# PytorchConnectomics/pytorch_connectomics

Hardware: AMD Instinct MI355X
Metric: voxels/s (train + sliding-window infer), MedNeXt-S 112^3 bf16 (higher is better)
Workload: dtype bf16; 1 GPU; Lucchi++ sliding-window inference (configs[1]): MedNeXt-S k3, 165x1024x768 volume, roi 112^3, overlap 0.5, bump blending, sw_batch_size 8, random-init weights; step = one whole-volume EagerSlidingWindowEngine call (TTA off); value = window-voxels/s; sw_batch_size=8, window_pipeline_streams=3

## Files before the change

### pytorch_connectomics_amd/csrc/pw_common.h

```cpp
#pragma once
#include "pytc_common.h"

namespace pytc {

template <typename TW>
struct Mma;

template <>
struct Mma<bf16_t> {
  static constexpr int EPL = 8;
  static constexpr int KSTEP = 32;
  typedef bf16x8_t frag_t;
  static __device__ __forceinline__ f32x4_t mma(frag_t a, frag_t b, f32x4_t c) {
    return __builtin_amdgcn_mfma_f32_16x16x32_bf16(a, b, c, 0, 0, 0);
  }
  static __device__ __forceinline__ frag_t from_floats(const float (&v)[8]) {
    f32x8_t f;
#pragma unroll
    for (int i = 0; i < 8; ++i) f[i] = v[i];
    return __builtin_convertvector(f, frag_t);
  }
};

template <>
// ... 79 lines not shown
    } else if (full) VecIO<TO, NCH>::load(resn + off, rv);
    else {
#pragma unroll
      for (int i = 0; i < NCH; ++i) rv[i] = (o0 + i < C_out) ? to_f32<TO>(resn[off + i]) : 0.f;
    }
    const float* cf = e.res_bias + (long)n * 3 * C_out + o0;
#pragma unroll
    for (int i = 0; i < NCH; ++i)
      if (o0 + i < C_out) v[i] = fmaf(cf[i], v[i], fmaf(cf[C_out + i], rv[i], cf[2 * C_out + i]));
    if (e.Go_w > 0) {
      const unsigned ur = (unsigned)orow, gw = (unsigned)e.Go_w, gh = (unsigned)e.Go_h;
      const unsigned tq = ur / gw;
      const int px = (int)(ur - tq * gw), pz = (int)(tq / gh), py = (int)(tq - (unsigned)pz * gh);
      if (px == 0 || py == 0 || pz == 0) return;
      const long crow = ((long)(pz - 1) * (e.Go_h - 1) + (py - 1)) * (e.Go_w - 1) + (px - 1);
      TO* yc = reinterpret_cast<TO*>(e.y) + ((long)n * (e.Go_d - 1) * (e.Go_h - 1) * (e.Go_w - 1) + crow) * C_out + o0;
      if (full) VecIO<TO, NCH>::store(yc, v);
      else {
#pragma unroll
        for (int i = 0; i < NCH; ++i)
          if (o0 + i < C_out) yc[i] = from_f32<TO>(v[i]);
      }
      return;
    }
  } else if (e.res_mode == PYTC_RES_UPSAMPLE) {
    int px, py, pz;
    if (pos) { pz = pos[0]; py = pos[1]; px = pos[2]; }
    else {
      const unsigned ur = (unsigned)orow, gw = (unsigned)e.Go_w, gh = (unsigned)e.Go_h;
      const unsigned t = ur / gw;
      px = (int)(ur - t * gw);
      pz = (int)(t / gh);
      py = (int)(t - (unsigned)pz * gh);
    }
    float sk[NCH];
    if (pre) {
#pragma unroll
      for (int i = 0; i < NCH; ++i) sk[i] = pre[i];
    } else if (full) VecIO<TO, NCH>::load(resn + off, sk);
    else {
#pragma unroll
      for (int i = 0; i < NCH; ++i) sk[i] = (o0 + i < C_out) ? to_f32<TO>(resn[off + i]) : 0.f;
    }
    if (px == 0 || py == 0 || pz == 0) {
#pragma unroll
      for (int i = 0; i < NCH; ++i) v[i] = sk[i];
    } else {
      const int oz = pz - 1, oy = py - 1, ox = px - 1;
      float rl[NCH];
      if (e.res_low && !((oz | oy | ox) & 1)) {
        const TO* rp = reinterpret_cast<const TO*>(e.res_low) +
                       ((((long)n * e.Gl_d + (oz >> 1)) * e.Gl_h + (oy >> 1)) * e.Gl_w + (ox >> 1)) * C_out + o0;
        if (full) VecIO<TO, NCH>::load(rp, rl);
        else {
#pragma unroll
          for (int i = 0; i < NCH; ++i) rl[i] = (o0 + i < C_out) ? to_f32<TO>(rp[i]) : 0.f;
        }
      } else {
#pragma unroll
        for (int i = 0; i < NCH; ++i) rl[i] = (e.res_bias && o0 + i < C_out) ? e.res_bias[o0 + i] : 0.f;
      }
#pragma unroll
      for (int i = 0; i < NCH; ++i) v[i] = v[i] + rl[i] + sk[i];
    }
  }
  if (full) {
    if constexpr (sizeof(TO) == 2 && NCH == 8) {
      if (e.nt) {
        f32x8_t f;
#pragma unroll
        for (int i = 0; i < 8; ++i) f[i] = v[i];
        __builtin_nontemporal_store(__builtin_convertvector(f, bf16x8_t), reinterpret_cast<bf16x8_t*>(yn + off));
        return;
      }
    }
    VecIO<TO, NCH>::store(yn + off, v);
  } else {
#pragma unroll
    for (int i = 0; i < NCH; ++i)
      if (o0 + i < C_out) yn[off + i] = from_f32<TO>(v[i]);
  }
}

template <typename TI, int EPL>
__device__ __forceinline__ void load_row_frag(const TI* __restrict__ row, int k0, int C_in, bool vec_ok,
                                              float (&v)[EPL]) {
  if (vec_ok && k0 + EPL <= C_in) {
    if constexpr (sizeof(TI) == 4 && EPL == 8) {
      float t0[4], t1[4];
      VecIO<float, 4>::load(reinterpret_cast<const float*>(row) + k0, t0);
      VecIO<float, 4>::load(reinterpret_cast<const float*>(row) + k0 + 4, t1);
#pragma unroll
      for (int i = 0; i < 4; ++i) { v[i] = t0[i]; v[4 + i] = t1[i]; }
    } else {
      VecIO<TI, EPL>::load(row + k0, v);
    }
  } else {
#pragma unroll
    for (int j = 0; j < EPL; ++j) v[j] = (k0 + j < C_in) ? to_f32<TI>(row[k0 + j]) : 0.f;
  }
}

template <int PER>
struct WarmRegs { unsigned int r[2 * PER]; };
template <int PER>
__device__ __forceinline__ void warm_l2(const void* base, long bytes, WarmRegs<PER>& w, int first) {
  const long lines = (bytes + 127) >> 7;
  const long lin = (long)blockIdx.z * gridDim.y * gridDim.x + (long)blockIdx.y * gridDim.x + blockIdx.x;
  const long total = (long)gridDim.x * gridDim.y * gridDim.z;
  const long per_xcd = (total + 7) >> 3;
  const long stride = per_xcd * blockDim.x;
  long l = (lin >> 3) * blockDim.x + threadIdx.x;
#pragma unroll
  for (int it = 0; it < PER; ++it, l += stride) {
    const long lc = l < lines ? l : lines - 1;
    const char* ptr = reinterpret_cast<const char*>(base) + (lc << 7);
    asm volatile("global_load_dword %0, %1, off" : "=v"(w.r[first + it]) : "v"(ptr) : "memory");
  }
}
template <int PER>
__device__ __forceinline__ void warm_l2_done(WarmRegs<PER>& w) {
  asm volatile("s_waitcnt vmcnt(0)" : : : "memory");
#pragma unroll
  for (int i = 0; i < 2 * PER; ++i) asm volatile("" : : "v"(w.r[i]) : "memory");
}

__device__ __forceinline__ float apply_act(float t, int act) {
  if (act == PYTC_ACT_GELU) return gelu_erf(t);
  if (act == PYTC_ACT_SIGMOID) return 1.f / (1.f + __expf(-t));
  if (act == PYTC_ACT_TANH) return tanhf(t);
  return t;
}

}
```

### pytorch_connectomics_amd/csrc/pw_mlp_chunk_kernels.hip

```cpp
#include "pw_common.h"

namespace pytc {

struct MlpChunkParams {
  const bf16_t* t;
  const float* ab;
  const bf16x8_t* w2;
  const float* b2;
  const h8_t* w3;
  const float* b3;
  EpiParams e;
  long rps;
  int N, C_in, C_hid, C_out, HC;
  long w2_stride;
};

__device__ __forceinline__ void chunk_glds16(const void* gsrc, unsigned lds_dst) {
  unsigned keep;
  asm volatile("s_mov_b32 %0, m0\n\ts_mov_b32 m0, %2\n\ts_nop 0\n\tglobal_load_lds_dwordx4 %1, off\n\ts_mov_b32 m0, %0"
               : "=&s"(keep) : "v"(gsrc), "s"(lds_dst) : "memory");
}

template <int KS_IN, int MO, int NW, int WPS>
__global__ void __launch_bounds__(NW * 64, WPS)
pw_mlp_chunk_kernel(MlpChunkParams p) {
  constexpr int NT = 2, CIN = KS_IN * 32, COUT = MO * 16;
  constexpr int PIECES = 2 * KS_IN + MO;
  constexpr int MINE = (PIECES + NW - 1) / NW;
  constexpr int NBUF = 3;
  extern __shared__ __attribute__((aligned(16))) unsigned char chunk_lds[];
  uint4* ring = reinterpret_cast<uint4*>(chunk_lds);
  float* lb2 = reinterpret_cast<float*>(chunk_lds + (size_t)NBUF * PIECES * 1024);
  float* lb3 = lb2 + p.C_hid;
  const int tid = threadIdx.x, lane = tid & 63;
  const int wave = __builtin_amdgcn_readfirstlane(tid >> 6);
  const int r = lane & 15, kb = lane >> 4;
  const int n = blockIdx.y;
  const bool folded = p.ab == nullptr;
  const long row0 = ((long)blockIdx.x * NW + wave) * (NT * 16);
  const bool with_res = p.e.res_mode != PYTC_RES_NONE;
  const bool ups = p.e.res_mode == PYTC_RES_UPSAMPLE;

  const unsigned char* w2img = reinterpret_cast<const unsigned char*>(p.w2 + (folded ? (long)n * p.w2_stride : 0L));
  const unsigned char* w3img = reinterpret_cast<const unsigned char*>(p.w3);
  const unsigned lbase = __builtin_amdgcn_readfirstlane((unsigned)(size_t)(__attribute__((address_space(3))) void*)ring);
  int mine = 0;
#pragma unroll
  for (int i = 0; i < MINE; ++i) mine += (wave + i * NW < PIECES) ? 1 : 0;
  auto request = [&](int hc) {
    const unsigned buf = lbase + (unsigned)((hc % NBUF) * PIECES) * 1024u;
#pragma unroll
    for (int i = 0; i < MINE; ++i) {
      const int pc = wave + i * NW;
      if (pc < PIECES) {
        const unsigned char* src = pc < 2 * KS_IN ? w2img + ((long)hc * (2 * KS_IN) + pc) * 1024
                                                  : w3img + ((long)(pc - 2 * KS_IN) * p.HC + hc) * 1024;
        chunk_glds16(src + lane * 16, buf + (unsigned)pc * 1024u);
      }
    }
  };

  long orow[NT];
#pragma unroll
  for (int nt = 0; nt < NT; ++nt) orow[nt] = row0 + nt * 16 + r;
  bf16x8_t bact[KS_IN][NT];
  const bf16_t* tn = p.t + (long)n * p.rps * CIN;
  uint4 raw[KS_IN][NT];
#pragma unroll
  for (int nt = 0; nt < NT; ++nt) {
    const long rr = orow[nt] < p.rps ? orow[nt] : p.rps - 1;
#pragma unroll
    for (int ks = 0; ks < KS_IN; ++ks) raw[ks][nt] = ld_stream(reinterpret_cast<const uint4*>(tn + rr * CIN + ks * 32 + kb * 8), p.e.nt);
  }
  {
    const float* b2 = p.b2 + (folded ? (long)n * p.C_hid : 0L);
    for (int i = tid; i < p.C_hid; i += NW * 64) lb2[i] = b2[i];
    if (tid < COUT) lb3[tid] = p.b3[tid];
  }
  request(0);
  if (p.HC > 1) request(1);
  const float* an = folded ? nullptr : p.ab + (long)n * 2 * CIN;
#pragma unroll
  for (int ks = 0; ks < KS_IN; ++ks) {
    if (folded) {
#pragma unroll
      for (int nt = 0; nt < NT; ++nt) bact[ks][nt] = __builtin_bit_cast(bf16x8_t, raw[ks][nt]);
    } else {
      const int k0 = ks * 32 + kb * 8;
      float av[8], bv[8];
      VecIO<float, 4>::load(an + k0, reinterpret_cast<float(&)[4]>(av[0]));
      VecIO<float, 4>::load(an + k0 + 4, reinterpret_cast<float(&)[4]>(av[4]));
      VecIO<float, 4>::load(an + CIN + k0, reinterpret_cast<float(&)[4]>(bv[0]));
      VecIO<float, 4>::load(an + CIN + k0 + 4, reinterpret_cast<float(&)[4]>(bv[4]));
#pragma unroll
      for (int nt = 0; nt < NT; ++nt) {
        float v[8];
        VecIO<bf16_t, 8>::load(reinterpret_cast<const bf16_t*>(&raw[ks][nt]), v);
#pragma unroll
        for (int j = 0; j < 8; ++j) v[j] = fmaf(v[j], av[j], bv[j]);
        bact[ks][nt] = Mma<bf16_t>::from_floats(v);
      }
    }
  }
#pragma unroll
  for (int ks = 0; ks < KS_IN; ++ks)
#pragma unroll
    for (int nt = 0; nt < NT; ++nt) asm volatile("" : "+v"(bact[ks][nt]));
  __syncthreads();
  f32x4_t acc2[MO][NT];
#pragma unroll
  for (int pr = 0; pr < MO / 2; ++pr) {
    const f32x4_t lo = *reinterpret_cast<const f32x4_t*>(lb3 + pr * 32 + kb * 8), hi = *reinterpret_cast<const f32x4_t*>(lb3 + pr * 32 + kb * 8 + 4);
#pragma unroll
    for (int nt = 0; nt < NT; ++nt) { acc2[2 * pr][nt] = lo; acc2[2 * pr + 1][nt] = hi; }
  }

  for (int hc = 0; hc < p.HC; ++hc) {
    if (hc + 1 < p.HC) {
      if (mine == 2) asm volatile("s_waitcnt vmcnt(2)" ::: "memory");
      else if (mine == 1) asm volatile("s_waitcnt vmcnt(1)" ::: "memory");
      else if (mine == 3) asm volatile("s_waitcnt vmcnt(3)" ::: "memory");
      else asm volatile("s_waitcnt vmcnt(0)" ::: "memory");
    } else {
      asm volatile("s_waitcnt vmcnt(0)" ::: "memory");
    }
    __syncthreads();
    if (hc + 2 < p.HC) request(hc + 2);
    const uint4* cb = ring + (size_t)(hc % NBUF) * PIECES * 64;
    const f32x4_t b2lo = *reinterpret_cast<const f32x4_t*>(lb2 + hc * 32 + kb * 8);
    const f32x4_t b2hi = *reinterpret_cast<const f32x4_t*>(lb2 + hc * 32 + kb * 8 + 4);
    f32x4_t acc1[2][NT];
#pragma unroll
    for (int nt = 0; nt < NT; ++nt) { acc1[0][nt] = b2lo; acc1[1][nt] = b2hi; }
#pragma unroll
    for (int mt = 0; mt < 2; ++mt) {
#pragma unroll
      for (int ks = 0; ks < KS_IN; ++ks) {
        const bf16x8_t a = __builtin_bit_cast(bf16x8_t, cb[(mt * KS_IN + ks) * 64 + lane]);
#pragma unroll
        for (int nt = 0; nt < NT; ++nt) acc1[mt][nt] = Mma<bf16_t>::mma(a, bact[ks][nt], acc1[mt][nt]);
      }
    }
    h8_t bhh[NT];
#pragma unroll
    for (int nt = 0; nt < NT; ++nt) {
      float gg[8];
#pragma unroll
      for (int j = 0; j < 4; ++j) { gg[j] = acc1[0][nt][j]; gg[4 + j] = acc1[1][nt][j]; }
      bhh[nt] = gelu_h8_from_f32(gg);
    }
#pragma unroll
    for (int mo = 0; mo < MO; ++mo) {
      const h8_t a = __builtin_bit_cast(h8_t, cb[(2 * KS_IN + mo) * 64 + lane]);
#pragma unroll
      for (int nt = 0; nt < NT; ++nt) acc2[mo][nt] = __builtin_amdgcn_mfma_f32_16x16x32_f16(a, bhh[nt], acc2[mo][nt], 0, 0, 0);
    }
  }

  if (row0 >= p.rps) return;
  int upos[NT][3];
  if (ups) {
    const unsigned ur = (unsigned)row0, gw = (unsigned)p.e.Go_w, gh = (unsigned)p.e.Go_h;
    const unsigned t0 = ur / gw;
    const int bx = (int)(ur - t0 * gw);
    const int bz = (int)(t0 / gh);
    const int by = (int)(t0 - (unsigned)bz * gh);
#pragma unroll
    for (int nt = 0; nt < NT; ++nt) {
      int px = bx + nt * 16 + r, py = by, pz = bz;
      while (px >= p.e.Go_w) { px -= p.e.Go_w; ++py; }
      while (py >= p.e.Go_h) { py -= p.e.Go_h; ++pz; }
      upos[nt][0] = pz; upos[nt][1] = py; upos[nt][2] = px;
    }
  }
#pragma unroll
  for (int pr = 0; pr < MO / 2; ++pr) {
#pragma unroll
    for (int nt = 0; nt < NT; ++nt) {
      if (orow[nt] >= p.rps) continue;
      float v[8];
#pragma unroll
      for (int j = 0; j < 4; ++j) { v[j] = acc2[2 * pr][nt][j]; v[4 + j] = acc2[2 * pr + 1][nt][j]; }
      finish_and_store<bf16_t, 8, false, COUT>(v, p.e, n, orow[nt], pr * 32 + kb * 8, nullptr, (with_res && ups) ? upos[nt] : nullptr);
    }
  }
}

template <int KS_IN, int MO, int NW, int WPS>
static void launch_mlp_chunk_v(const MlpChunkParams& p, hipStream_t s) {
  auto kern = &pw_mlp_chunk_kernel<KS_IN, MO, NW, WPS>;
  const size_t lds = (size_t)3 * (2 * KS_IN + MO) * 1024 + (size_t)(p.C_hid + MO * 16) * 4;
  if (!ensure_dynamic_lds(reinterpret_cast<const void*>(kern), 160 * 1024, "pw_mlp_chunk")) return;
  const long wg_rows = (long)NW * 32;
  dim3 grid((unsigned)((p.rps + wg_rows - 1) / wg_rows), (unsigned)p.N), block(NW * 64);
  hipLaunchKernelGGL(kern, grid, block, lds, s, p);
}

template <int KS_IN, int MO>
static void launch_mlp_chunk(const MlpChunkParams& p, int variant, hipStream_t s) {
  if (variant == 0) variant = (KS_IN == 8) ? 1 : 3;
  switch (variant) {
    case 2: launch_mlp_chunk_v<KS_IN, MO, 12, 3>(p, s); break;
    case 3: launch_mlp_chunk_v<KS_IN, MO, 8, 4>(p, s); break;
    case 4: launch_mlp_chunk_v<KS_IN, MO, 16, 4>(p, s); break;
    default: launch_mlp_chunk_v<KS_IN, MO, 8, 2>(p, s); break;
  }
}

}

using namespace pytc;

extern "C" int pytc_pw_mlp_chunk_supported(int C_in, int C_hid, int C_out) {
  if (C_in % 32 || C_hid % 32 || C_out % 32) return 0;
  const int ks = C_in / 32, mo = C_out / 16;
  const bool shape = (ks == 2 && (mo == 2 || mo == 4 || mo == 8)) || (ks == 4 && mo == 4) || (ks == 4 && mo == 8) || (ks == 8 && mo == 8);
  return (shape && C_hid >= 64 && C_hid <= 8192) ? 1 : 0;
}

extern "C" int pytc_pw_mlp_chunk_fwd(const pytc_mlp_args* a, void* stream) {
  PYTC_REQUIRE(a && a->t && (a->ab || a->per_sample) && a->w2_packed && a->w3_packed && a->b2 && a->b3 && a->y, "pw_mlp_chunk: null pointer");
  PYTC_REQUIRE(!(a->ab && a->per_sample), "pw_mlp_chunk: per-sample (norm-folded) expand operands come without an affine");
  PYTC_REQUIRE(a->w3_format == PYTC_W3_F16, "pw_mlp_chunk: the projection image must be fp16 (pytc_pw_pack_weight_paired_f16)");
  PYTC_REQUIRE(a->N >= 1 && a->rows_per_sample >= 1, "pw_mlp_chunk: bad shape");
  if (!pytc_pw_mlp_chunk_supported(a->C_in, a->C_hid, a->C_out)) {
    set_error("pw_mlp_chunk: no chunk-streamed kernel for C_in=%d C_hid=%d C_out=%d", a->C_in, a->C_hid, a->C_out);
    return PYTC_ERR_UNSUPPORTED;
  }
  PYTC_REQUIRE(a->res_mode == PYTC_RES_NONE || a->res, "pw_mlp_chunk: residual mode without residual pointer");
  PYTC_REQUIRE(a->res_mode == PYTC_RES_NONE || a->res_mode == PYTC_RES_ADD || a->res_mode == PYTC_RES_UPSAMPLE, "pw_mlp_chunk: residual mode");
  MlpChunkParams p{};
  p.t = (const bf16_t*)a->t; p.ab = a->ab; p.w2 = (const bf16x8_t*)a->w2_packed; p.b2 = a->b2;
  p.w3 = (const h8_t*)a->w3_packed; p.b3 = a->b3;
  p.rps = a->rows_per_sample; p.N = a->N; p.C_in = a->C_in; p.C_hid = a->C_hid; p.C_out = a->C_out; p.HC = a->C_hid / 32;
  p.w2_stride = (long)(a->C_hid / 16) * (a->C_in / 32) * 64;
  p.e.res = a->res; p.e.res_low = a->res_low; p.e.res_bias = a->res_bias; p.e.y = a->y;
  p.e.rps_out = a->rows_per_sample; p.e.C_out = a->C_out; p.e.res_mode = a->res_mode;
  p.e.nt = 0;
  p.e.Go_d = p.e.Go_h = p.e.Go_w = p.e.Gl_d = p.e.Gl_h = p.e.Gl_w = 0;
  if (a->res_mode == PYTC_RES_UPSAMPLE) {
    PYTC_REQUIRE((long)a->Di * a->Hi * a->Wi == a->rows_per_sample && !(a->Di & 1) && !(a->Hi & 1) && !(a->Wi & 1) &&
                 a->rows_per_sample < (1L << 31), "pw_mlp_chunk: RES_UPSAMPLE needs the (even) output grid");
    p.e.Go_d = a->Di; p.e.Go_h = a->Hi; p.e.Go_w = a->Wi;
    p.e.Gl_d = a->Di / 2; p.e.Gl_h = a->Hi / 2; p.e.Gl_w = a->Wi / 2;
  }
  hipStream_t s = (hipStream_t)stream;
  const int ks = a->C_in / 32, mo = a->C_out / 16;
  const int variant = tuning_get(K_mlp_chunk_variant);
  if (ks == 2 && mo == 2) launch_mlp_chunk<2, 2>(p, variant, s);
  else if (ks == 2 && mo == 4) launch_mlp_chunk<2, 4>(p, variant, s);
  else if (ks == 2 && mo == 8) launch_mlp_chunk<2, 8>(p, variant, s);
  else if (ks == 4 && mo == 4) launch_mlp_chunk<4, 4>(p, variant, s);
  else if (ks == 4 && mo == 8) launch_mlp_chunk<4, 8>(p, variant, s);
  else launch_mlp_chunk<8, 8>(p, variant, s);
  PYTC_LAUNCH_CHECK("pw_mlp_chunk");
  return PYTC_OK;
}
```

### pytorch_connectomics_amd/csrc/pw_mlp_lds_kernels.hip

```cpp
#include <mutex>

#include "pw_common.h"

namespace pytc {

struct MlpLdsParams {
  const bf16_t* t;
  const float* ab;
  const bf16x8_t* w2;
  const float* b2;
  const h8_t* w3;
  const float* b3;
  EpiParams e;
  long rps;
  int N, C_in, C_hid, C_out, HC;
  long w2_stride;
};

template <int KS_IN, int MO, int NT>
struct LdsTile {
  uint4 raw[KS_IN][NT];
  uint4 res[MO / 2][NT];
};

template <int KS_IN, int MO, int NT>
__device__ __forceinline__ void lds_tile_load(LdsTile<KS_IN, MO, NT>& T, const MlpLdsParams& p, int n, long row0, int r, int kb,
                                              bool with_res) {
  const bf16_t* tn = p.t + (long)n * p.rps * (KS_IN * 32);
#pragma unroll
  for (int nt = 0; nt < NT; ++nt) {
    const long o = row0 + nt * 16 + r;
    const long rr = o < p.rps ? o : p.rps - 1;
#pragma unroll
    for (int ks = 0; ks < KS_IN; ++ks) T.raw[ks][nt] = ld_stream(reinterpret_cast<const uint4*>(tn + rr * (KS_IN * 32) + ks * 32 + kb * 8), p.e.nt);
  }
  if (with_res) {
    const bf16_t* resn = reinterpret_cast<const bf16_t*>(p.e.res) + (long)n * p.rps * (MO * 16);
#pragma unroll
    for (int nt = 0; nt < NT; ++nt) {
      const long o = row0 + nt * 16 + r;
      const long rr = o < p.rps ? o : p.rps - 1;
#pragma unroll
      for (int pr = 0; pr < MO / 2; ++pr) T.res[pr][nt] = ld_stream(reinterpret_cast<const uint4*>(resn + rr * (MO * 16) + pr * 32 + kb * 8), p.e.nt);
    }
  }
}

template <int KS_IN, int MO, int NT, int NWAVES, int WPS>
__global__ void __launch_bounds__(NWAVES * 64, WPS)
pw_mlp_lds_kernel(MlpLdsParams p) {
  constexpr int CIN = KS_IN * 32, COUT = MO * 16;
  extern __shared__ __attribute__((aligned(16))) unsigned char lds_raw[];
  bf16x8_t* lw2 = reinterpret_cast<bf16x8_t*>(lds_raw);
  h8_t* lw3 = reinterpret_cast<h8_t*>(lds_raw + (size_t)p.C_hid * CIN * 2);
  float* lb2 = reinterpret_cast<float*>(lds_raw + (size_t)p.C_hid * (CIN + COUT) * 2);
  const int tid = threadIdx.x, wave = tid >> 6, lane = tid & 63;
  const int r = lane & 15, kb = lane >> 4;
  const bool folded = p.ab == nullptr;
  const int n_w2 = p.C_hid * CIN / 8, n_w3 = COUT * p.C_hid / 8;
  for (int i = tid; i < n_w3; i += NWAVES * 64) lw3[i] = p.w3[i];
  const long Ts = (p.rps + NT * 16 - 1) / (NT * 16);
  const long G = Ts * p.N;
  const long g_end = G * (blockIdx.x + 1) / gridDim.x;
  long g = G * blockIdx.x / gridDim.x;
  const bool with_res = p.e.res_mode != PYTC_RES_NONE;
  const bool ups = p.e.res_mode == PYTC_RES_UPSAMPLE;
  int staged = -1;

  while (g < g_end) {
    const int n = (int)(g / Ts);
    const long seg_end = min(g_end, (long)(n + 1) * Ts);
    if (staged < 0 || folded) {
      __syncthreads();
      const bf16x8_t* src = p.w2 + (folded ? (long)n * p.w2_stride : 0L);
      for (int i = tid; i < n_w2; i += NWAVES * 64) lw2[i] = src[i];
      const float* b2 = p.b2 + (folded ? (long)n * p.C_hid : 0L);
      for (int i = tid; i < p.C_hid; i += NWAVES * 64) lb2[i] = b2[i];
      staged = n;
      __syncthreads();
    }
    const float* an = folded ? nullptr : p.ab + (long)n * 2 * CIN;
    const long t_base = (long)n * Ts;

    for (long gt = g + wave; gt < seg_end; gt += NWAVES) {
      const long row0 = (gt - t_base) * (NT * 16);
      LdsTile<KS_IN, MO, NT> cur;
      lds_tile_load(cur, p, n, row0, r, kb, with_res);
      long orow[NT];
#pragma unroll
      for (int nt = 0; nt < NT; ++nt) orow[nt] = row0 + nt * 16 + r;

      bf16x8_t bact[KS_IN][NT];
#pragma unroll
      for (int ks = 0; ks < KS_IN; ++ks) {
        if (folded) {
#pragma unroll
          for (int nt = 0; nt < NT; ++nt) bact[ks][nt] = __builtin_bit_cast(bf16x8_t, cur.raw[ks][nt]);
        } else {
          const int k0 = ks * 32 + kb * 8;
          float av[8], bv[8];
          VecIO<float, 4>::load(an + k0, reinterpret_cast<float(&)[4]>(av[0]));
          VecIO<float, 4>::load(an + k0 + 4, reinterpret_cast<float(&)[4]>(av[4]));
          VecIO<float, 4>::load(an + CIN + k0, reinterpret_cast<float(&)[4]>(bv[0]));
          VecIO<float, 4>::load(an + CIN + k0 + 4, reinterpret_cast<float(&)[4]>(bv[4]));
#pragma unroll
          for (int nt = 0; nt < NT; ++nt) {
            float v[8];
            VecIO<bf16_t, 8>::load(reinterpret_cast<const bf16_t*>(&cur.raw[ks][nt]), v);
#pragma unroll
            for (int j = 0; j < 8; ++j) v[j] = fmaf(v[j], av[j], bv[j]);
            bact[ks][nt] = Mma<bf16_t>::from_floats(v);
          }
        }
      }
      f32x4_t acc2[MO][NT];
#pragma unroll
      for (int pr = 0; pr < MO / 2; ++pr) {
        float b[8];
        VecIO<float, 4>::load(p.b3 + pr * 32 + kb * 8, reinterpret_cast<float(&)[4]>(b[0]));
        VecIO<float, 4>::load(p.b3 + pr * 32 + kb * 8 + 4, reinterpret_cast<float(&)[4]>(b[4]));
#pragma unroll
        for (int nt = 0; nt < NT; ++nt) {
          acc2[2 * pr][nt] = f32x4_t{b[0], b[1], b[2], b[3]};
          acc2[2 * pr + 1][nt] = f32x4_t{b[4], b[5], b[6], b[7]};
        }
      }
      for (int hc = 0; hc < p.HC; ++hc) {
        const f32x4_t b2lo = *reinterpret_cast<const f32x4_t*>(lb2 + hc * 32 + kb * 8);
        const f32x4_t b2hi = *reinterpret_cast<const f32x4_t*>(lb2 + hc * 32 + kb * 8 + 4);
        f32x4_t acc1[2][NT];
#pragma unroll
        for (int nt = 0; nt < NT; ++nt) { acc1[0][nt] = b2lo; acc1[1][nt] = b2hi; }
#pragma unroll
        for (int mt = 0; mt < 2; ++mt) {
#pragma unroll
          for (int ks = 0; ks < KS_IN; ++ks) {
            const bf16x8_t a = lw2[((hc * 2 + mt) * KS_IN + ks) * 64 + lane];
#pragma unroll
            for (int nt = 0; nt < NT; ++nt) acc1[mt][nt] = Mma<bf16_t>::mma(a, bact[ks][nt], acc1[mt][nt]);
          }
        }
        h8_t bhh[NT];
#pragma unroll
        for (int nt = 0; nt < NT; ++nt) {
          float gg[8];
#pragma unroll
          for (int j = 0; j < 4; ++j) { gg[j] = acc1[0][nt][j]; gg[4 + j] = acc1[1][nt][j]; }
          bhh[nt] = gelu_h8_from_f32(gg);
        }
#pragma unroll
        for (int mo = 0; mo < MO; ++mo) {
          const h8_t a = lw3[(mo * p.HC + hc) * 64 + lane];
#pragma unroll
          for (int nt = 0; nt < NT; ++nt) acc2[mo][nt] = __builtin_amdgcn_mfma_f32_16x16x32_f16(a, bhh[nt], acc2[mo][nt], 0, 0, 0);
        }
      }
      int upos[NT][3];
      if (ups) {
        const unsigned ur = (unsigned)row0, gw = (unsigned)p.e.Go_w, gh = (unsigned)p.e.Go_h;
        const unsigned t0 = ur / gw;
        const int bx = (int)(ur - t0 * gw);
        const int bz = (int)(t0 / gh);
        const int by = (int)(t0 - (unsigned)bz * gh);
#pragma unroll
        for (int nt = 0; nt < NT; ++nt) {
          int px = bx + nt * 16 + r, py = by, pz = bz;
          while (px >= p.e.Go_w) { px -= p.e.Go_w; ++py; }
          while (py >= p.e.Go_h) { py -= p.e.Go_h; ++pz; }
          upos[nt][0] = pz; upos[nt][1] = py; upos[nt][2] = px;
        }
      }
#pragma unroll
      for (int pr = 0; pr < MO / 2; ++pr) {
#pragma unroll
        for (int nt = 0; nt < NT; ++nt) {
          if (orow[nt] >= p.rps) continue;
          float v[8];
#pragma unroll
          for (int j = 0; j < 4; ++j) { v[j] = acc2[2 * pr][nt][j]; v[4 + j] = acc2[2 * pr + 1][nt][j]; }
          if (with_res) {
            float pre[8];
            VecIO<bf16_t, 8>::load(reinterpret_cast<const bf16_t*>(&cur.res[pr][nt]), pre);
            finish_and_store<bf16_t, 8, false, COUT>(v, p.e, n, orow[nt], pr * 32 + kb * 8, pre, ups ? upos[nt] : nullptr);
          } else {
            finish_and_store<bf16_t, 8, false, COUT>(v, p.e, n, orow[nt], pr * 32 + kb * 8, nullptr, nullptr);
          }
        }
      }
    }
    g = seg_end;
  }
}

template <int KS_IN, int MO, int NT, int NWAVES, int WPS>
static void launch_mlp_lds_v(const MlpLdsParams& p, size_t lds, hipStream_t s) {
  auto kern = &pw_mlp_lds_kernel<KS_IN, MO, NT, NWAVES, WPS>;
  if (!ensure_dynamic_lds(reinterpret_cast<const void*>(kern), 160 * 1024, "pw_mlp_lds")) return;
  const long tiles = ((p.rps + NT * 16 - 1) / (NT * 16)) * p.N;
  const int by_lds = (int)((160 * 1024) / lds), by_waves = WPS * 4 / NWAVES;
  const int per_cu = by_lds < by_waves ? (by_lds < 1 ? 1 : by_lds) : by_waves;
  long blocks = 256L * per_cu;
  const long need = (tiles + NWAVES - 1) / NWAVES;
  if (blocks > need) blocks = need;
  hipLaunchKernelGGL(kern, dim3((unsigned)blocks), dim3(NWAVES * 64), lds, s, p);
}

template <int KS_IN, int MO, int NT>
static void launch_mlp_lds(const MlpLdsParams& p, int variant, hipStream_t s) {
  const size_t lds = (size_t)p.C_hid * (p.C_in + p.C_out) * 2 + (size_t)p.C_hid * 4;
  if (variant == 0) variant = (KS_IN == 4 && MO == 8) ? 3 : (MO == 2 ? 2 : 4);
  switch (variant) {
    case 1: launch_mlp_lds_v<KS_IN, MO, NT, 8, 4>(p, lds, s); break;
    case 2: launch_mlp_lds_v<KS_IN, MO, NT, 16, 4>(p, lds, s); break;
    case 3: launch_mlp_lds_v<KS_IN, MO, NT, 8, 2>(p, lds, s); break;
    default: launch_mlp_lds_v<KS_IN, MO, NT, 12, 3>(p, lds, s); break;
  }
}

}

using namespace pytc;

extern "C" int pytc_pw_mlp_lds_supported(int C_in, int C_hid, int C_out) {
  if (C_in % 32 || C_hid % 32 || C_out % 32) return 0;
  const int ks = C_in / 32, mo = C_out / 16;
  const bool shape = (ks == 2 && mo == 2) || (ks == 2 && mo == 4) || (ks == 4 && mo == 4) || (ks == 4 && mo == 8);
  const size_t lds = (size_t)C_hid * (C_in + C_out) * 2 + (size_t)C_hid * 4;
  return (shape && lds <= 160 * 1024) ? 1 : 0;
}

extern "C" int pytc_pw_mlp_lds_fwd(const pytc_mlp_args* a, void* stream) {
  PYTC_REQUIRE(a && a->t && (a->ab || a->per_sample) && a->w2_packed && a->w3_packed && a->b2 && a->b3 && a->y, "pw_mlp_lds: null pointer");
  PYTC_REQUIRE(!(a->ab && a->per_sample), "pw_mlp_lds: per-sample (norm-folded) expand operands come without an affine");
  PYTC_REQUIRE(a->w3_format == PYTC_W3_F16, "pw_mlp_lds: the projection image must be fp16 (pytc_pw_pack_weight_paired_f16)");
  PYTC_REQUIRE(a->N >= 1 && a->rows_per_sample >= 1, "pw_mlp_lds: bad shape");
  if (!pytc_pw_mlp_lds_supported(a->C_in, a->C_hid, a->C_out)) {
    set_error("pw_mlp_lds: no LDS-resident kernel for C_in=%d C_hid=%d C_out=%d", a->C_in, a->C_hid, a->C_out);
    return PYTC_ERR_UNSUPPORTED;
  }
  PYTC_REQUIRE(a->res_mode == PYTC_RES_NONE || a->res, "pw_mlp_lds: residual mode without residual pointer");
  MlpLdsParams p{};
  p.t = (const bf16_t*)a->t; p.ab = a->ab; p.w2 = (const bf16x8_t*)a->w2_packed; p.b2 = a->b2;
  p.w3 = (const h8_t*)a->w3_packed; p.b3 = a->b3;
  p.rps = a->rows_per_sample; p.N = a->N; p.C_in = a->C_in; p.C_hid = a->C_hid; p.C_out = a->C_out; p.HC = a->C_hid / 32;
  p.w2_stride = (long)(a->C_hid / 16) * (a->C_in / 32) * 64;
  p.e.res = a->res; p.e.res_low = a->res_low; p.e.res_bias = a->res_bias; p.e.y = a->y;
  p.e.rps_out = a->rows_per_sample; p.e.C_out = a->C_out; p.e.res_mode = a->res_mode;
  p.e.nt = 0;
  p.e.Go_d = p.e.Go_h = p.e.Go_w = p.e.Gl_d = p.e.Gl_h = p.e.Gl_w = 0;
  if (a->res_mode == PYTC_RES_UPSAMPLE) {
    PYTC_REQUIRE((long)a->Di * a->Hi * a->Wi == a->rows_per_sample && !(a->Di & 1) && !(a->Hi & 1) && !(a->Wi & 1) &&
                 a->rows_per_sample < (1L << 31), "pw_mlp_lds: RES_UPSAMPLE needs the (even) output grid");
    p.e.Go_d = a->Di; p.e.Go_h = a->Hi; p.e.Go_w = a->Wi;
    p.e.Gl_d = a->Di / 2; p.e.Gl_h = a->Hi / 2; p.e.Gl_w = a->Wi / 2;
  }
  hipStream_t s = (hipStream_t)stream;
  const int ks = a->C_in / 32, mo = a->C_out / 16;
  const int variant = tuning_get(K_mlp_lds_variant);
  if (ks == 2 && mo == 2) launch_mlp_lds<2, 2, 2>(p, variant, s);
  else if (ks == 2 && mo == 4) launch_mlp_lds<2, 4, 2>(p, variant, s);
  else if (ks == 4 && mo == 4) launch_mlp_lds<4, 4, 2>(p, variant, s);
  else launch_mlp_lds<4, 8, 2>(p, variant, s);
  PYTC_LAUNCH_CHECK("pw_mlp_lds");
  return PYTC_OK;
}
```

### pytorch_connectomics_amd/csrc/pytc_common.h

```cpp
#pragma once
#include <hip/hip_runtime.h>
#include <stdint.h>
#include <stdio.h>
#include <string.h>

#include "../../include/pytc_hip.h"

namespace pytc {

typedef __bf16 bf16_t;
typedef __bf16 bf16x2_t __attribute__((ext_vector_type(2)));
typedef __bf16 bf16x4_t __attribute__((ext_vector_type(4)));
typedef __bf16 bf16x8_t __attribute__((ext_vector_type(8)));
typedef float f32x2_t __attribute__((ext_vector_type(2)));
typedef float f32x4_t __attribute__((ext_vector_type(4)));
typedef float f32x8_t __attribute__((ext_vector_type(8)));
typedef float f32x16_t __attribute__((ext_vector_type(16)));
typedef short s16x8_t __attribute__((ext_vector_type(8)));

constexpr int WAVE = 64;

void set_error(const char* fmt, ...);
int hip_fail(hipError_t e, const char* what);
bool ensure_dynamic_lds(const void* kernel, size_t bytes, const char* what);
bool take_launch_failure();

#define PYTC_REQUIRE(cond, ...)                     \
  do {                                              \
    if (!(cond)) {                                  \
      pytc::set_error(__VA_ARGS__);                 \
      return PYTC_ERR_INVALID;                      \
    }                                               \
  } while (0)

#define PYTC_LAUNCH_CHECK(name)                                  \
  do {                                                           \
    if (pytc::take_launch_failure()) return PYTC_ERR_HIP;        \
    hipError_t e_ = hipGetLastError();                           \
    if (e_ != hipSuccess) return pytc::hip_fail(e_, name);       \
  } while (0)

#define PYTC_KNOBS(X)                                                                                                             \
  X(channel_act_flat, 1, "channel activation of contiguous NDHWC tensors as a flat 16-byte stream; 0 = the per-voxel kernel")      \
  X(conv_wgrad_mfma, 1, "dense-conv weight gradient on the matrix cores (bf16); 0 = the VALU kernel")                              \
  X(dw_wgrad_march, 1, "depthwise K = 3 / stride 1 weight gradient as a z-march; 0 = the vector / generic kernels")                \
  X(dw_wgrad_vec, 1, "depthwise K = 3 weight gradient with 16-byte channel vectors; 0 = the generic kernel")                       \
  X(dwconvT_tile, 1, "transposed depthwise conv at C = 64 / 128 (bf16) as one tile of input cells per workgroup; 0 = cell kernel") \
  X(dwconv_march_h16, 1, "VALU z-march depthwise conv: packed-f16 in-plane partial sums; 0 = fp32 taps")                           \
  X(dwconv_mfma, 1, "bf16 stride-1 K = 3 depthwise forward (and the fused block) on the matrix cores; 0 = the VALU z-march")       \
  X(dwconv_mfma_variant, 0, "matrix-core depthwise conv: bit 0 = hi + lo weight halves, bit 1 = two planes in flight, not three")  \
  X(dwconv_s2_march, 1, "stride-2 K = 3 depthwise conv at C = 32 / 64 (bf16) as a z-march over an LDS ring; 0 = gather kernel")    \
  X(elementwise_vec, 1, "16-byte vector forms of the norm-apply / elementwise training kernels; 0 = the scalar kernels")           \
  X(mixer_bwd_rc_slot_div, 1, "recomputing mixer backward: divide the slot count (fewer, longer slots)")                           \
  X(mlp_chunk_variant, 0, "chunked-hidden mixer (pw_mlp_chunk_kernels.hip): tile shape of the launch")                             \
  X(mlp_dma, 1, "level-0 mixer with DMA-prefetched row tiles (pw_mlp_dma_kernel); 0 = one tile per wave")                          \
  X(mlp_dma_rows, 1 << 20, "fewest rows of a launch that takes the DMA mixer")                                                     \
  X(mlp_dma_wgs, 0, "DMA mixer: workgroups per sample; 0 = chosen from the row count")                                             \
  X(mlp_lds_variant, 0, "LDS-resident mixer (pw_mlp_lds_kernels.hip): tile shape of the launch")                                   \
  X(norm_bwd_from_wgrad_flat, 1, "GroupNorm-backward epilogue of the expand weight gradient as one flat kernel; 0 = chunked")      \
  X(pw_gemm_rows, 0, "LDS-tiled 1x1 GEMM: 64 / 128 forces the rows per workgroup; 0 = by problem size")                            \
  X(pw_thin, 1, "plain 1x1 convs with one input / few output channels on the thin kernels; 0 = the generic kernel")                \
  X(wgrad_dgrad_fused, 1, "projecting conv's weight gradient and the GELU-backward data gradient in one kernel; 0 = two launches")  \
  X(wgrad_small_split, 1, "matrix-core 1x1 weight gradient: more, shorter row slots when the launch would leave CUs idle")         \
  X(wgrad_valu, 0, "1: 1x1 weight gradient on the VALU kernel instead of the matrix cores")                                        \
  X(wgrad_whole_rounds, 1, "matrix-core 1x1 weight gradient: round the slot count down to whole rounds of resident workgroups")

enum Knob {
#define PYTC_KNOB_ENUM(name, dflt, doc) K_##name,
  PYTC_KNOBS(PYTC_KNOB_ENUM)
#undef PYTC_KNOB_ENUM
  K_COUNT
};
int tuning_get(Knob k);

template <typename T, int VEC>
struct VecIO;

template <int VEC>
struct VecIO<float, VEC> {
  typedef float vec_t __attribute__((ext_vector_type(VEC)));
  static __device__ __forceinline__ void load(const float* p, float (&v)[VEC]) {
    vec_t t = *reinterpret_cast<const vec_t*>(p);
#pragma unroll
    for (int i = 0; i < VEC; ++i) v[i] = t[i];
  }
  static __device__ __forceinline__ void store(float* p, const float (&v)[VEC]) {
    vec_t t;
#pragma unroll
    for (int i = 0; i < VEC; ++i) t[i] = v[i];
    *reinterpret_cast<vec_t*>(p) = t;
  }
};
template <>
struct VecIO<float, 1> {
  static __device__ __forceinline__ void load(const float* p, float (&v)[1]) { v[0] = *p; }
  static __device__ __forceinline__ void store(float* p, const float (&v)[1]) { *p = v[0]; }
};

template <int VEC>
struct VecIO<bf16_t, VEC> {
  typedef __bf16 vec_t __attribute__((ext_vector_type(VEC)));
  typedef float fvec_t __attribute__((ext_vector_type(VEC)));
  static __device__ __forceinline__ void load(const bf16_t* p, float (&v)[VEC]) {
    vec_t t = *reinterpret_cast<const vec_t*>(p);
    fvec_t f = __builtin_convertvector(t, fvec_t);
#pragma unroll
    for (int i = 0; i < VEC; ++i) v[i] = f[i];
  }
  static __device__ __forceinline__ void store(bf16_t* p, const float (&v)[VEC]) {
    fvec_t f;
#pragma unroll
    for (int i = 0; i < VEC; ++i) f[i] = v[i];
    *reinterpret_cast<vec_t*>(p) = __builtin_convertvector(f, vec_t);
  }
};
template <>
struct VecIO<bf16_t, 1> {
  static __device__ __forceinline__ void load(const bf16_t* p, float (&v)[1]) { v[0] = (float)*p; }
  static __device__ __forceinline__ void store(bf16_t* p, const float (&v)[1]) { *p = (bf16_t)v[0]; }
};

template <typename T>
__device__ __forceinline__ float to_f32(T v) { return (float)v; }
template <typename T>
__device__ __forceinline__ T from_f32(float v) { return (T)v; }

__device__ __forceinline__ float wave_sum(float v) {
#pragma unroll
  for (int o = 32; o > 0; o >>= 1) v += __shfl_xor(v, o, 64);
  return v;
}

__device__ __forceinline__ float gelu_erf(float x) {
  const float az = fabsf(x) * 0.70710678118654752440f;
  const float t = __builtin_amdgcn_rcpf(fmaf(0.3275911f, az, 1.0f));
  float p = fmaf(t, 1.061405429f, -1.453152027f);
  p = fmaf(t, p, 1.421413741f);
  p = fmaf(t, p, -0.284496736f);
  p = fmaf(t, p, 0.254829592f);
  p *= t;
  const float pe = p * __builtin_amdgcn_exp2f(-az * az * 1.44269504088896340736f);
  const float one_plus_erf = x < 0.f ? pe : 2.0f - pe;
  return 0.5f * x * one_plus_erf;
}
// ... 96 lines not shown
```

Baseline: 1.839 billion voxels/s.

## Prefetch upsample-epilogue skip and low-res operands early in mixer kernels

In the LDS-resident and chunked mixer kernels, the RES_UPSAMPLE epilogue now issues its skip-row loads and low-resolution residual gathers before the GEMM work. The low-resolution rows go straight into per-wave LDS landing slots via global_load_lds. Grid coordinates are advanced incrementally with a cursor instead of per-row divisions. The goal is to hide epilogue memory latency behind the matrix-core work. The cost is extra LDS and registers, which the launcher gates so resident workgroup count does not drop; it also adds a default-on knob.

```diff
diff --git a/pytorch_connectomics_amd/csrc/pw_common.h b/pytorch_connectomics_amd/csrc/pw_common.h
--- a/pytorch_connectomics_amd/csrc/pw_common.h
+++ b/pytorch_connectomics_amd/csrc/pw_common.h
@@ -185,6 +185,72 @@
   }
 }
 
+
+struct GridStep {
+  int z, y, x;
+  __device__ __forceinline__ GridStep(unsigned rows, int gh, int gw) {
+    const unsigned t = rows / (unsigned)gw;
+    x = (int)(rows - t * (unsigned)gw);
+    z = (int)(t / (unsigned)gh);
+    y = (int)(t - (unsigned)z * (unsigned)gh);
+  }
+};
+
+struct UpsampleCursor {
+  int pz, py, px;
+  static __device__ __forceinline__ void add(int& z, int& y, int& x, const GridStep& s, int gh, int gw) {
+    x += s.x;
+    const bool cx = x >= gw;
+    x = cx ? x - gw : x;
+    y += s.y + (cx ? 1 : 0);
+    const bool cy = y >= gh;
+    y = cy ? y - gh : y;
+    z += s.z + (cy ? 1 : 0);
+  }
+  __device__ __forceinline__ void seek(unsigned row, int gh, int gw) {
+    const unsigned t = row / (unsigned)gw;
+    px = (int)(row - t * (unsigned)gw);
+    pz = (int)(t / (unsigned)gh);
+    py = (int)(t - (unsigned)pz * (unsigned)gh);
+  }
+  __device__ __forceinline__ void advance(const GridStep& s, int gh, int gw) { add(pz, py, px, s, gh, gw); }
+  template <int NT>
+  __device__ __forceinline__ unsigned tile(unsigned (&low)[NT], const GridStep& s16, int gh, int gw, int gl_h, int gl_w, unsigned rows_low) const {
+    int z = pz, y = py, x = px;
+    unsigned flags = 0;
+#pragma unroll
+    for (int nt = 0; nt < NT; ++nt) {
+      if (nt) add(z, y, x, s16, gh, gw);
+      flags |= ((z == 0 || y == 0 || x == 0) ? 1u : 0u) << (2 * nt);
+      flags |= (unsigned)(z & y & x & 1) << (2 * nt + 1);
+      const unsigned lz = (unsigned)max(z - 1, 0) >> 1, ly = (unsigned)max(y - 1, 0) >> 1, lx = (unsigned)max(x - 1, 0) >> 1;
+      low[nt] = min((lz * (unsigned)gl_h + ly) * (unsigned)gl_w + lx, rows_low - 1u);
+    }
+    return flags;
+  }
+};
+
+__device__ __forceinline__ void upsample_finish_store(float (&v)[8], bf16_t* yrow, const uint4& sk_raw, const uint4& low_raw,
+                                                      const float (&rb)[8], bool face, bool on_low, int nt) {
+  float sk[8], rl[8];
+  VecIO<bf16_t, 8>::load(reinterpret_cast<const bf16_t*>(&sk_raw), sk);
+  VecIO<bf16_t, 8>::load(reinterpret_cast<const bf16_t*>(&low_raw), rl);
+#pragma unroll
+  for (int i = 0; i < 8; ++i) {
+    const float r = on_low ? rl[i] : rb[i];
+    const float s = v[i] + r + sk[i];
+    v[i] = face ? sk[i] : s;
+  }
+  if (nt) {
+    f32x8_t f;
+#pragma unroll
+    for (int i = 0; i < 8; ++i) f[i] = v[i];
+    __builtin_nontemporal_store(__builtin_convertvector(f, bf16x8_t), reinterpret_cast<bf16x8_t*>(yrow));
+    return;
+  }
+  VecIO<bf16_t, 8>::store(yrow, v);
+}
+
 template <typename TI, int EPL>
 __device__ __forceinline__ void load_row_frag(const TI* __restrict__ row, int k0, int C_in, bool vec_ok,
                                               float (&v)[EPL]) {
diff --git a/pytorch_connectomics_amd/csrc/pw_mlp_chunk_kernels.hip b/pytorch_connectomics_amd/csrc/pw_mlp_chunk_kernels.hip
--- a/pytorch_connectomics_amd/csrc/pw_mlp_chunk_kernels.hip
+++ b/pytorch_connectomics_amd/csrc/pw_mlp_chunk_kernels.hip
@@ -1,3 +1,5 @@
+#include <algorithm>
+
 #include "pw_common.h"
 
 namespace pytc {
@@ -21,7 +23,7 @@
                : "=&s"(keep) : "v"(gsrc), "s"(lds_dst) : "memory");
 }
 
-template <int KS_IN, int MO, int NW, int WPS>
+template <int KS_IN, int MO, int NW, int WPS, bool UPF = false>
 __global__ void __launch_bounds__(NW * 64, WPS)
 pw_mlp_chunk_kernel(MlpChunkParams p) {
   constexpr int NT = 2, CIN = KS_IN * 32, COUT = MO * 16;
@@ -32,6 +34,8 @@
   uint4* ring = reinterpret_cast<uint4*>(chunk_lds);
   float* lb2 = reinterpret_cast<float*>(chunk_lds + (size_t)NBUF * PIECES * 1024);
   float* lb3 = lb2 + p.C_hid;
+  float* lrb = lb3 + COUT;
+  constexpr int LAND = (MO / 2) * NT * 64;
   const int tid = threadIdx.x, lane = tid & 63;
   const int wave = __builtin_amdgcn_readfirstlane(tid >> 6);
   const int r = lane & 15, kb = lane >> 4;
@@ -72,10 +76,41 @@
 #pragma unroll
     for (int ks = 0; ks < KS_IN; ++ks) raw[ks][nt] = ld_stream(reinterpret_cast<const uint4*>(tn + rr * CIN + ks * 32 + kb * 8), p.e.nt);
   }
+  uint4 skip[UPF ? MO / 2 : 1][NT];
+  unsigned uflags = 0;
+  const uint4* land = reinterpret_cast<const uint4*>(lrb + COUT) + (UPF ? wave * LAND : 0);
+  if constexpr (UPF) {
+    const bf16_t* resn = reinterpret_cast<const bf16_t*>(p.e.res) + (long)n * p.rps * COUT;
+#pragma unroll
+    for (int nt = 0; nt < NT; ++nt) {
+      const long rr = orow[nt] < p.rps ? orow[nt] : p.rps - 1;
+#pragma unroll
+      for (int pr = 0; pr < MO / 2; ++pr) skip[pr][nt] = ld_stream(reinterpret_cast<const uint4*>(resn + rr * COUT + pr * 32 + kb * 8), p.e.nt);
+    }
+    const unsigned rows_low = (unsigned)p.e.Gl_d * (unsigned)p.e.Gl_h * (unsigned)p.e.Gl_w;
+    const GridStep s16(16u, p.e.Go_h, p.e.Go_w);
+    UpsampleCursor pos;
+    pos.seek((unsigned)row0 + (unsigned)r, p.e.Go_h, p.e.Go_w);
+    unsigned lr[NT];
+    uflags = pos.tile(lr, s16, p.e.Go_h, p.e.Go_w, p.e.Gl_h, p.e.Gl_w, rows_low);
+    if (p.e.res_low) {
+      const bf16_t* lown = reinterpret_cast<const bf16_t*>(p.e.res_low) + (long)n * rows_low * COUT;
+      const unsigned land_lds = __builtin_amdgcn_readfirstlane((unsigned)(size_t)(__attribute__((address_space(3))) const void*)land);
+#pragma unroll
+      for (int nt = 0; nt < NT; ++nt) {
+        const bf16_t* lrow = lown + (long)lr[nt] * COUT + kb * 8;
+#pragma unroll
+        for (int pr = 0; pr < MO / 2; ++pr) chunk_glds16(lrow + pr * 32, land_lds + (unsigned)((pr * NT + nt) * 64) * 16u);
+      }
+    }
+  }
   {
     const float* b2 = p.b2 + (folded ? (long)n * p.C_hid : 0L);
     for (int i = tid; i < p.C_hid; i += NW * 64) lb2[i] = b2[i];
     if (tid < COUT) lb3[tid] = p.b3[tid];
+    if constexpr (UPF) {
+      if (tid < COUT) lrb[tid] = p.e.res_bias ? p.e.res_bias[tid] : 0.f;
+    }
   }
   request(0);
   if (p.HC > 1) request(1);
@@ -158,6 +193,26 @@
   }
 
   if (row0 >= p.rps) return;
+  if constexpr (UPF) {
+    bf16_t* yn = reinterpret_cast<bf16_t*>(p.e.y) + (long)n * p.rps * COUT;
+    const bool has_low = p.e.res_low != nullptr;
+#pragma unroll
+    for (int pr = 0; pr < MO / 2; ++pr) {
+      const f32x4_t lo = *reinterpret_cast<const f32x4_t*>(lrb + pr * 32 + kb * 8), hi = *reinterpret_cast<const f32x4_t*>(lrb + pr * 32 + kb * 8 + 4);
+      const float rb[8] = {lo[0], lo[1], lo[2], lo[3], hi[0], hi[1], hi[2], hi[3]};
+#pragma unroll
+      for (int nt = 0; nt < NT; ++nt) {
+        if (orow[nt] >= p.rps) continue;
+        float v[8];
+#pragma unroll
+        for (int j = 0; j < 4; ++j) { v[j] = acc2[2 * pr][nt][j]; v[4 + j] = acc2[2 * pr + 1][nt][j]; }
+        const bool on_low = has_low && ((uflags >> (2 * nt + 1)) & 1u);
+        const uint4 low = on_low ? land[(pr * NT + nt) * 64 + lane] : uint4{0u, 0u, 0u, 0u};
+        upsample_finish_store(v, yn + orow[nt] * COUT + pr * 32 + kb * 8, skip[pr][nt], low, rb, (uflags >> (2 * nt)) & 1u, on_low, p.e.nt);
+      }
+    }
+    return;
+  }
   int upos[NT][3];
   if (ups) {
     const unsigned ur = (unsigned)row0, gw = (unsigned)p.e.Go_w, gh = (unsigned)p.e.Go_h;
@@ -187,13 +242,26 @@
 }
 
 template <int KS_IN, int MO, int NW, int WPS>
-static void launch_mlp_chunk_v(const MlpChunkParams& p, hipStream_t s) {
-  auto kern = &pw_mlp_chunk_kernel<KS_IN, MO, NW, WPS>;
-  const size_t lds = (size_t)3 * (2 * KS_IN + MO) * 1024 + (size_t)(p.C_hid + MO * 16) * 4;
+constexpr bool kChunkUpfOk = MO <= 4 || WPS == 2;
+
+template <int KS_IN, int MO, int NW, int WPS, bool UPF>
+static void launch_mlp_chunk_u(const MlpChunkParams& p, size_t lds, hipStream_t s) {
+  auto kern = &pw_mlp_chunk_kernel<KS_IN, MO, NW, WPS, UPF>;
   if (!ensure_dynamic_lds(reinterpret_cast<const void*>(kern), 160 * 1024, "pw_mlp_chunk")) return;
   const long wg_rows = (long)NW * 32;
   dim3 grid((unsigned)((p.rps + wg_rows - 1) / wg_rows), (unsigned)p.N), block(NW * 64);
   hipLaunchKernelGGL(kern, grid, block, lds, s, p);
+}
+
+template <int KS_IN, int MO, int NW, int WPS>
+static void launch_mlp_chunk_v(const MlpChunkParams& p, hipStream_t s) {
+  const size_t lds = (size_t)3 * (2 * KS_IN + MO) * 1024 + (size_t)(p.C_hid + MO * 16) * 4;
+  const size_t lds_up = lds + (size_t)MO * 16 * 4 + (size_t)NW * MO * 1024;
+  constexpr int by_waves = WPS * 4 / NW;
+  const int want = (int)std::min<size_t>(160 * 1024 / lds, by_waves), have = (int)std::min<size_t>(160 * 1024 / lds_up, by_waves);
+  if (kChunkUpfOk<KS_IN, MO, NW, WPS> && p.e.res_mode == PYTC_RES_UPSAMPLE && tuning_get(K_up_epilogue_prefetch) != 0 && have >= want && have >= 1)
+    launch_mlp_chunk_u<KS_IN, MO, NW, WPS, true>(p, lds_up, s);
+  else launch_mlp_chunk_u<KS_IN, MO, NW, WPS, false>(p, lds, s);
 }
 
 template <int KS_IN, int MO>
diff --git a/pytorch_connectomics_amd/csrc/pw_mlp_lds_kernels.hip b/pytorch_connectomics_amd/csrc/pw_mlp_lds_kernels.hip
--- a/pytorch_connectomics_amd/csrc/pw_mlp_lds_kernels.hip
+++ b/pytorch_connectomics_amd/csrc/pw_mlp_lds_kernels.hip
@@ -1,3 +1,4 @@
+#include <algorithm>
 #include <mutex>
 
 #include "pw_common.h"
@@ -46,7 +47,13 @@
   }
 }
 
-template <int KS_IN, int MO, int NT, int NWAVES, int WPS>
+__device__ __forceinline__ void lds_glds16(const void* gsrc, unsigned lds_dst) {
+  unsigned keep;
+  asm volatile("s_mov_b32 %0, m0\n\ts_mov_b32 m0, %2\n\ts_nop 0\n\tglobal_load_lds_dwordx4 %1, off\n\ts_mov_b32 m0, %0"
+               : "=&s"(keep) : "v"(gsrc), "s"(lds_dst) : "memory");
+}
+
+template <int KS_IN, int MO, int NT, int NWAVES, int WPS, bool UPF = false>
 __global__ void __launch_bounds__(NWAVES * 64, WPS)
 pw_mlp_lds_kernel(MlpLdsParams p) {
   constexpr int CIN = KS_IN * 32, COUT = MO * 16;
@@ -59,6 +66,15 @@
   const bool folded = p.ab == nullptr;
   const int n_w2 = p.C_hid * CIN / 8, n_w3 = COUT * p.C_hid / 8;
   for (int i = tid; i < n_w3; i += NWAVES * 64) lw3[i] = p.w3[i];
+  float* lrb = lb2 + p.C_hid;
+  if constexpr (UPF) {
+    if (tid < COUT) lrb[tid] = p.e.res_bias ? p.e.res_bias[tid] : 0.f;
+  }
+  const GridStep s16(16u, UPF ? p.e.Go_h : 1, UPF ? p.e.Go_w : 1), stile((unsigned)(NWAVES * NT * 16), UPF ? p.e.Go_h : 1, UPF ? p.e.Go_w : 1);
+  const unsigned rows_low = (unsigned)p.e.Gl_d * (unsigned)p.e.Gl_h * (unsigned)p.e.Gl_w;
+  constexpr int LAND = (MO / 2) * NT * 64;
+  const uint4* land = reinterpret_cast<const uint4*>(lrb + COUT) + (UPF ? __builtin_amdgcn_readfirstlane(wave) * LAND : 0);
+  const unsigned land_lds = UPF ? __builtin_amdgcn_readfirstlane((unsigned)(size_t)(__attribute__((address_space(3))) const void*)land) : 0u;
   const long Ts = (p.rps + NT * 16 - 1) / (NT * 16);
   const long G = Ts * p.N;
   const long g_end = G * (blockIdx.x + 1) / gridDim.x;
@@ -81,11 +97,30 @@
     }
     const float* an = folded ? nullptr : p.ab + (long)n * 2 * CIN;
     const long t_base = (long)n * Ts;
+    UpsampleCursor pos;
+    const bf16_t* lown = nullptr;
+    if constexpr (UPF) {
+      pos.seek((unsigned)((g + wave - t_base) * (NT * 16)) + (unsigned)r, p.e.Go_h, p.e.Go_w);
+      if (p.e.res_low) lown = reinterpret_cast<const bf16_t*>(p.e.res_low) + (long)n * rows_low * COUT;
+    }
 
     for (long gt = g + wave; gt < seg_end; gt += NWAVES) {
       const long row0 = (gt - t_base) * (NT * 16);
       LdsTile<KS_IN, MO, NT> cur;
       lds_tile_load(cur, p, n, row0, r, kb, with_res);
+      unsigned uflags = 0;
+      if constexpr (UPF) {
+        unsigned lr[NT];
+        uflags = pos.tile(lr, s16, p.e.Go_h, p.e.Go_w, p.e.Gl_h, p.e.Gl_w, rows_low);
+        if (lown) {
+#pragma unroll
+          for (int nt = 0; nt < NT; ++nt) {
+            const bf16_t* lrow = lown + (long)lr[nt] * COUT + kb * 8;
+#pragma unroll
+            for (int pr = 0; pr < MO / 2; ++pr) lds_glds16(lrow + pr * 32, land_lds + (unsigned)((pr * NT + nt) * 64) * 16u);
+          }
+        }
+      }
       long orow[NT];
 #pragma unroll
       for (int nt = 0; nt < NT; ++nt) orow[nt] = row0 + nt * 16 + r;
@@ -155,6 +190,32 @@
           for (int nt = 0; nt < NT; ++nt) acc2[mo][nt] = __builtin_amdgcn_mfma_f32_16x16x32_f16(a, bhh[nt], acc2[mo][nt], 0, 0, 0);
         }
       }
+      if constexpr (UPF) {
+        bf16_t* yn = reinterpret_cast<bf16_t*>(p.e.y) + (long)n * p.rps * COUT;
+        asm volatile("s_waitcnt vmcnt(0)" ::: "memory");
+        __builtin_amdgcn_wave_barrier();
+#pragma unroll
+        for (int pr = 0; pr < MO / 2; ++pr) {
+          float rb[8];
+          VecIO<float, 4>::load(lrb + pr * 32 + kb * 8, reinterpret_cast<float(&)[4]>(rb[0]));
+          VecIO<float, 4>::load(lrb + pr * 32 + kb * 8 + 4, reinterpret_cast<float(&)[4]>(rb[4]));
+#pragma unroll
+          for (int nt = 0; nt < NT; ++nt) {
+            const long o = row0 + nt * 16 + r;
+            if (o >= p.rps) continue;
+            float v[8];
+#pragma unroll
+            for (int j = 0; j < 4; ++j) { v[j] = acc2[2 * pr][nt][j]; v[4 + j] = acc2[2 * pr + 1][nt][j]; }
+            const bool on_low = lown != nullptr && ((uflags >> (2 * nt + 1)) & 1u);
+            const uint4 low = on_low ? land[(pr * NT + nt) * 64 + lane] : uint4{0u, 0u, 0u, 0u};
+            upsample_finish_store(v, yn + o * COUT + pr * 32 + kb * 8, cur.res[pr][nt], low, rb, (uflags >> (2 * nt)) & 1u, on_low, p.e.nt);
+          }
+        }
+        asm volatile("s_waitcnt lgkmcnt(0)" ::: "memory");
+        __builtin_amdgcn_wave_barrier();
+        pos.advance(stile, p.e.Go_h, p.e.Go_w);
+        continue;
+      }
       int upos[NT][3];
       if (ups) {
         const unsigned ur = (unsigned)row0, gw = (unsigned)p.e.Go_w, gh = (unsigned)p.e.Go_h;
@@ -192,9 +253,9 @@
   }
 }
 
-template <int KS_IN, int MO, int NT, int NWAVES, int WPS>
-static void launch_mlp_lds_v(const MlpLdsParams& p, size_t lds, hipStream_t s) {
-  auto kern = &pw_mlp_lds_kernel<KS_IN, MO, NT, NWAVES, WPS>;
+template <int KS_IN, int MO, int NT, int NWAVES, int WPS, bool UPF>
+static void launch_mlp_lds_u(const MlpLdsParams& p, size_t lds, hipStream_t s) {
+  auto kern = &pw_mlp_lds_kernel<KS_IN, MO, NT, NWAVES, WPS, UPF>;
   if (!ensure_dynamic_lds(reinterpret_cast<const void*>(kern), 160 * 1024, "pw_mlp_lds")) return;
   const long tiles = ((p.rps + NT * 16 - 1) / (NT * 16)) * p.N;
   const int by_lds = (int)((160 * 1024) / lds), by_waves = WPS * 4 / NWAVES;
@@ -203,6 +264,19 @@
   const long need = (tiles + NWAVES - 1) / NWAVES;
   if (blocks > need) blocks = need;
   hipLaunchKernelGGL(kern, dim3((unsigned)blocks), dim3(NWAVES * 64), lds, s, p);
+}
+
+template <int KS_IN, int MO, int NWAVES, int WPS>
+constexpr bool kLdsUpfOk = MO == 2 || WPS == 2 || (KS_IN == 2 && WPS == 3);
+
+template <int KS_IN, int MO, int NT, int NWAVES, int WPS>
+static void launch_mlp_lds_v(const MlpLdsParams& p, size_t lds, hipStream_t s) {
+  const size_t lds_up = lds + (size_t)MO * 16 * 4 + (size_t)NWAVES * (MO / 2) * NT * 1024;
+  constexpr int by_waves = WPS * 4 / NWAVES;
+  const int want = (int)std::min<size_t>(160 * 1024 / lds, by_waves), have = (int)std::min<size_t>(160 * 1024 / lds_up, by_waves);
+  if (kLdsUpfOk<KS_IN, MO, NWAVES, WPS> && p.e.res_mode == PYTC_RES_UPSAMPLE && tuning_get(K_up_epilogue_prefetch) != 0 && have >= want && have >= 1)
+    launch_mlp_lds_u<KS_IN, MO, NT, NWAVES, WPS, true>(p, lds_up, s);
+  else launch_mlp_lds_u<KS_IN, MO, NT, NWAVES, WPS, false>(p, lds, s);
 }
 
 template <int KS_IN, int MO, int NT>
diff --git a/pytorch_connectomics_amd/csrc/pytc_common.h b/pytorch_connectomics_amd/csrc/pytc_common.h
--- a/pytorch_connectomics_amd/csrc/pytc_common.h
+++ b/pytorch_connectomics_amd/csrc/pytc_common.h
@@ -60,6 +60,7 @@
   X(norm_bwd_from_wgrad_flat, 1, "GroupNorm-backward epilogue of the expand weight gradient as one flat kernel; 0 = chunked")      \
   X(pw_gemm_rows, 0, "LDS-tiled 1x1 GEMM: 64 / 128 forces the rows per workgroup; 0 = by problem size")                            \
   X(pw_thin, 1, "plain 1x1 convs with one input / few output channels on the thin kernels; 0 = the generic kernel")                \
+  X(up_epilogue_prefetch, 1, "RES_UPSAMPLE epilogue of the LDS-resident / chunked mixers: operands requested early; 0 = after")    \
   X(wgrad_dgrad_fused, 1, "projecting conv's weight gradient and the GELU-backward data gradient in one kernel; 0 = two launches")  \
   X(wgrad_small_split, 1, "matrix-core 1x1 weight gradient: more, shorter row slots when the launch would leave CUs idle")         \
   X(wgrad_valu, 0, "1: 1x1 weight gradient on the VALU kernel instead of the matrix cores")                                        \
```

Result: no change. 1.846 billion voxels/s, median of 6 (+0.4%).
